# microsoft/singleshotpose

Hardware: NVIDIA H100
Metric: images/sec fwd+bwd+SGD (416x416, yolo-pose.cfg) (higher is better)
Workload: dtype f16x2-split operands, f32 accumulate (fwd); f16 operands, f32 accumulate (bwd)

## Files before the change

singleshotpose_b200/csrc/conv_tc.cu:

```cuda
#include "ssp_common.cuh"
#include "tmap.cuh"

namespace ssp {

struct ConvTcParams {
  CUtensorMap tmA[2];
  CUtensorMap tmB[2];
  long long m_rows;
  long long store_rows;
  int m_tiles, n_tiles;
  int kc_per_tap, cin, taps;
  int shifts[9];
  int Wp, HpWp;
  int cout, bn, n_terms;
  int fmt;
  int stages, stage_bytes, b_bytes;
  float* out;
  long long out_ld;
  const float* bias;
  double* stat_sum;
  double* stat_sq;
  int epi;
  FusedAct fa;
  int splits;
  long long slab_elems;
};

static constexpr int kABytes = 128 * 128;
static constexpr int kMaxStages = 8;
static constexpr int kAccCols = 1024;
static constexpr int kThreads = 256;
static constexpr int kSplitMinKblocks = 8;

template <bool FUSED, int BN, int BF, int NT, bool SPLIT = false>
__global__ void __launch_bounds__(kThreads, 1) conv_tc_kernel(const __grid_constant__ ConvTcParams p) {
  extern __shared__ __align__(1024) uint8_t smem_raw[];
  uint8_t* smem = (uint8_t*)(((uintptr_t)smem_raw + 1023) & ~(uintptr_t)1023);
  uint8_t* stage_base = smem;
  double* acc_sum = (double*)(smem + (size_t)p.stages * p.stage_bytes);
  double* acc_sq = acc_sum + kAccCols;
  float* stg = (float*)(acc_sq + kAccCols);
  uint64_t* full_bar = (uint64_t*)((uint8_t*)stg + kStageRowsBytes);
  uint64_t* empty_bar = full_bar + kMaxStages;

  const int warp = threadIdx.x >> 5;
  const int lane = threadIdx.x & 31;
  const int total_tiles = p.m_tiles * p.n_tiles;
  const int kblocks = p.taps * p.kc_per_tap;

  if (warp == 0 && lane == 0) {
    tma_prefetch_desc(&p.tmA[0]);
    tma_prefetch_desc(&p.tmB[0]);
    if (p.n_terms == 3) { tma_prefetch_desc(&p.tmA[1]); tma_prefetch_desc(&p.tmB[1]); }
  }
  if (warp == 1 && lane == 0) {
    for (int s = 0; s < p.stages; s++) { mbar_init(&full_bar[s], 1); mbar_init(&empty_bar[s], 4); }
    fence_barrier_init();
  }
  if (p.epi == EPI_STATS)
    for (int i = threadIdx.x; i < 2 * kAccCols; i += kThreads) acc_sum[i] = 0.0;
  __syncthreads();

  if (warp == 0) {
    if (lane == 0) {
      int stage = 0; uint32_t phase = 0;
      const uint32_t tx = (uint32_t)(p.n_terms == 3 ? 2 : 1) * (uint32_t)(kABytes + p.b_bytes);
      if constexpr (SPLIT) {
        for (int t = blockIdx.x; t < total_tiles * p.splits; t += gridDim.x) {
          const int tile = t / p.splits, sp = t % p.splits;
          const int m0 = (tile / p.n_tiles) * 128, n0 = (tile % p.n_tiles) * p.bn;
          const int kb1 = (int)((long long)(sp + 1) * kblocks / p.splits);
          for (int kb = (int)((long long)sp * kblocks / p.splits); kb < kb1; kb++) {
            const int tap = kb / p.kc_per_tap, kc = kb - tap * p.kc_per_tap;
            const int arow = m0 + p.shifts[tap];
            mbar_wait(&empty_bar[stage], phase ^ 1);
            uint8_t* sa = stage_base + (size_t)stage * p.stage_bytes;
            mbar_expect_tx(&full_bar[stage], tx);
            const int kcol_b = tap * p.cin + kc * 64;
            tma_load_2d(sa, &p.tmA[0], &full_bar[stage], kc * 64, arow);
            if (p.n_terms == 3) {
              tma_load_2d(sa + kABytes, &p.tmA[1], &full_bar[stage], kc * 64, arow);
              tma_load_2d(sa + 2 * kABytes, &p.tmB[0], &full_bar[stage], kcol_b, n0);
              tma_load_2d(sa + 2 * kABytes + p.b_bytes, &p.tmB[1], &full_bar[stage], kcol_b, n0);
            } else {
              tma_load_2d(sa + kABytes, &p.tmB[0], &full_bar[stage], kcol_b, n0);
            }
            if (++stage == p.stages) { stage = 0; phase ^= 1; }
          }
        }
      } else {
      for (int t = blockIdx.x; t < total_tiles; t += gridDim.x) {
        const int mt = t / p.n_tiles, nt = t % p.n_tiles;
        const int m0 = mt * 128, n0 = nt * p.bn;
        for (int tap = 0; tap < p.taps; tap++) {
          const int arow = m0 + p.shifts[tap];
          for (int kc = 0; kc < p.kc_per_tap; kc++) {
            mbar_wait(&empty_bar[stage], phase ^ 1);
            uint8_t* sa = stage_base + (size_t)stage * p.stage_bytes;
            mbar_expect_tx(&full_bar[stage], tx);
            const int kcol_b = tap * p.cin + kc * 64;
            tma_load_2d(sa, &p.tmA[0], &full_bar[stage], kc * 64, arow);
            if (p.n_terms == 3) {
              tma_load_2d(sa + kABytes, &p.tmA[1], &full_bar[stage], kc * 64, arow);
              tma_load_2d(sa + 2 * kABytes, &p.tmB[0], &full_bar[stage], kcol_b, n0);
              tma_load_2d(sa + 2 * kABytes + p.b_bytes, &p.tmB[1], &full_bar[stage], kcol_b, n0);
            } else {
              tma_load_2d(sa + kABytes, &p.tmB[0], &full_bar[stage], kcol_b, n0);
            }
            if (++stage == p.stages) { stage = 0; phase ^= 1; }
          }
        }
      }
      }
    }
  } else if (warp >= 4) {
    const int et = threadIdx.x - 128;
    int stage = 0; uint32_t phase = 0;
    float acc[2][BN / 2];
    const int items = SPLIT ? total_tiles * p.splits : total_tiles;
    for (int t = blockIdx.x; t < items; t += gridDim.x) {
      int tile = t, sp = 0, kb0 = 0, kb1 = kblocks;
      if constexpr (SPLIT) {
        tile = t / p.splits; sp = t % p.splits;
        kb0 = (int)((long long)sp * kblocks / p.splits); kb1 = (int)((long long)(sp + 1) * kblocks / p.splits);
      }
      const int mt = tile / p.n_tiles, nt = tile % p.n_tiles;
      int prev = -1;
      for (int kb = kb0; kb < kb1; kb++) {
        mbar_wait(&full_bar[stage], phase);
        const uint32_t sa = smem_u32(stage_base + (size_t)stage * p.stage_bytes);
        const uint32_t a_hi = sa, a_lo = sa + kABytes;
        const uint32_t b_hi = (NT == 3) ? sa + 2 * kABytes : sa + kABytes;
        const uint32_t b_lo = b_hi + p.b_bytes;
        wgmma_fence();
#pragma unroll
        for (int k = 0; k < 4; k++) {
          const uint64_t dbh = gmma_desc_k_sw128(b_hi + k * 32);
#pragma unroll
          for (int h = 0; h < 2; h++) {
            const uint64_t dah = gmma_desc_k_sw128(a_hi + h * 8192 + k * 32);
            const int sd = (kb > kb0 || k > 0) ? 1 : 0;
            if constexpr (NT == 3) {
              wgmma_f32<BN, 0, 0, BF>(acc[h], gmma_desc_k_sw128(a_lo + h * 8192 + k * 32), dbh, sd);
              wgmma_f32<BN, 0, 0, BF>(acc[h], dah, gmma_desc_k_sw128(b_lo + k * 32), 1);
              wgmma_f32<BN, 0, 0, BF>(acc[h], dah, dbh, 1);
            } else {
              wgmma_f32<BN, 0, 0, BF>(acc[h], dah, dbh, sd);
            }
          }
        }
        wgmma_commit();
        wgmma_wait<1>();
        if (prev >= 0 && lane == 0) mbar_arrive(&empty_bar[prev]);
        prev = stage;
        if (++stage == p.stages) { stage = 0; phase ^= 1; }
      }
      wgmma_wait<0>();
      if (prev >= 0 && lane == 0) mbar_arrive(&empty_bar[prev]);

      const long long m = (long long)mt * 128 + et;
      const int n0 = nt * p.bn;
      bool valid = false;
      if (m < p.m_rows) {
        const int rem = (int)(m % p.HpWp);
        valid = (rem / p.Wp >= 1) && (rem % p.Wp >= 1);
      }
      float* orow = (p.out && p.epi != EPI_F16) ? p.out + m * p.out_ld : nullptr;
      const bool can_store = m < p.store_rows;
#pragma unroll
      for (int ch = 0; ch < BN / 32; ch++) {
        float v[32];
        acc_rows_32<BN>(acc, ch, stg, et, v);
        const int c0 = n0 + ch * 32;
        if constexpr (SPLIT) {
          if (can_store) {
            float* o = p.out + sp * p.slab_elems + m * p.out_ld;
            if (c0 + 32 <= p.cout) {
#pragma unroll
              for (int j = 0; j < 32; j += 4) *reinterpret_cast<float4*>(o + c0 + j) = make_float4(v[j], v[j + 1], v[j + 2], v[j + 3]);
            } else {
#pragma unroll
              for (int j = 0; j < 32; j++) if (c0 + j < p.cout) o[c0 + j] = v[j];
            }
          }
          continue;
        }
        if constexpr (FUSED) {
          if (valid && c0 + 32 <= p.cout) {
            uint32_t ph[16], pl[16];
#pragma unroll
            for (int j = 0; j < 32; j += 2) {
              uint16_t h0, l0, h1, l1;
              float z0 = fmaf(v[j], __ldg(p.fa.scale + c0 + j), __ldg(p.fa.shift + c0 + j));
              float z1 = fmaf(v[j + 1], __ldg(p.fa.scale + c0 + j + 1), __ldg(p.fa.shift + c0 + j + 1));
              z0 = z0 > 0.f ? z0 : z0 * p.fa.slope; z1 = z1 > 0.f ? z1 : z1 * p.fa.slope;
              split_f16(z0, h0, l0); split_f16(z1, h1, l1);
              ph[j >> 1] = h0 | ((uint32_t)h1 << 16); pl[j >> 1] = l0 | ((uint32_t)l1 << 16);
            }
            uint4* dh = reinterpret_cast<uint4*>(p.fa.d_hi + m * p.fa.d_ld + p.fa.d_c0 + c0);
            uint4* dl = reinterpret_cast<uint4*>(p.fa.d_lo + m * p.fa.d_ld + p.fa.d_c0 + c0);
#pragma unroll
            for (int j = 0; j < 4; j++) {
              dh[j] = make_uint4(ph[4 * j], ph[4 * j + 1], ph[4 * j + 2], ph[4 * j + 3]);
              dl[j] = make_uint4(pl[4 * j], pl[4 * j + 1], pl[4 * j + 2], pl[4 * j + 3]);
            }
          }
          continue;
        }
        if (p.epi == EPI_BIAS) {
#pragma unroll
          for (int j = 0; j < 32; j++) if (c0 + j < p.cout) v[j] += __ldg(p.bias + c0 + j);
        }
        if (p.epi == EPI_F16) {
          if (can_store) {
            uint16_t* o16 = reinterpret_cast<uint16_t*>(p.out) + m * p.out_ld + c0;
            if (c0 + 32 <= p.cout) {
              uint32_t pk[16];
#pragma unroll
              for (int j = 0; j < 16; j++) pk[j] = cvt_f32_to_16(v[2 * j], FMT_F16) | ((uint32_t)cvt_f32_to_16(v[2 * j + 1], FMT_F16) << 16);
#pragma unroll
              for (int j = 0; j < 4; j++) reinterpret_cast<uint4*>(o16)[j] = make_uint4(pk[4 * j], pk[4 * j + 1], pk[4 * j + 2], pk[4 * j + 3]);
            } else {
#pragma unroll
              for (int j = 0; j < 32; j++) if (c0 + j < p.cout) o16[j] = cvt_f32_to_16(v[j], FMT_F16);
            }
          }
        } else if (can_store && p.epi != 3) {
          if (c0 + 32 <= p.cout) {
#pragma unroll
            for (int j = 0; j < 32; j += 4)
              *reinterpret_cast<float4*>(orow + c0 + j) = make_float4(v[j], v[j + 1], v[j + 2], v[j + 3]);
          } else {
#pragma unroll
            for (int j = 0; j < 32; j++) if (c0 + j < p.cout) orow[c0 + j] = v[j];
          }
        }
        if (p.epi == EPI_STATS) {
          float s1[32], s2[32];
#pragma unroll
          for (int j = 0; j < 32; j++) { const float x = valid ? v[j] : 0.f; s1[j] = x; s2[j] = x * x; }
          const float cs = warp_transpose_sum32(s1, lane);
          const float cq = warp_transpose_sum32(s2, lane);
          if (c0 + lane < p.cout) {
            atomicAdd(&acc_sum[c0 + lane], (double)cs);
            atomicAdd(&acc_sq[c0 + lane], (double)cq);
          }
        }
      }
    }
    if (p.epi == EPI_STATS) {
      epi_bar();
      for (int c = et; c < p.cout; c += 128) {
        const double a = acc_sum[c], b = acc_sq[c];
        if (a != 0.0 || b != 0.0) { atomicAdd(p.stat_sum + c, a); atomicAdd(p.stat_sq + c, b); }
      }
    }
  }
}

template <bool FUSED, int BF, int NT, bool SPLIT = false>
static int launch_conv_tc(const ConvTcParams& p, int grid, int smem_bytes, cudaStream_t stream) {
  static int configured = 0;
  if (!configured) {
    cudaError_t e = cudaSuccess;
    for (auto k : {conv_tc_kernel<FUSED, 32, BF, NT, SPLIT>, conv_tc_kernel<FUSED, 64, BF, NT, SPLIT>, conv_tc_kernel<FUSED, 128, BF, NT, SPLIT>})
      if (e == cudaSuccess) e = cudaFuncSetAttribute(k, cudaFuncAttributeMaxDynamicSharedMemorySize, 227 * 1024);
    if (e != cudaSuccess) return fail_cuda(e, __FILE__, __LINE__);
    configured = 1;
  }
  if (p.bn == 32) conv_tc_kernel<FUSED, 32, BF, NT, SPLIT><<<grid, kThreads, smem_bytes, stream>>>(p);
  else if (p.bn == 64) conv_tc_kernel<FUSED, 64, BF, NT, SPLIT><<<grid, kThreads, smem_bytes, stream>>>(p);
  else conv_tc_kernel<FUSED, 128, BF, NT, SPLIT><<<grid, kThreads, smem_bytes, stream>>>(p);
  SSP_CHECK_LAUNCH();
  return SSP_OK;
}

static int g_num_sms = 0;

static void tile_geometry(int N, int H, int W, int taps, int cin, int cout, long long* tiles, int* kblocks) {
  const int bn = cout > 64 ? 128 : ((cout + 31) / 32) * 32;
  *tiles = ((Geom{N, H, W}.m_rows() + 127) / 128) * (long long)((cout + bn - 1) / bn);
  *kblocks = taps * ((cin + 63) / 64);
}

int conv_splitk_count(int N, int H, int W, int taps, int cin, int cout, int num_sms) {
  if (N <= 0 || H <= 0 || W <= 0 || (taps != 1 && taps != 9) || cin <= 0 || cout <= 0 || num_sms <= 0)
    return fail_msg(SSP_ERR_ARG, "ssp_conv_splitk_count: bad argument");
  long long tiles; int kblocks;
  tile_geometry(N, H, W, taps, cin, cout, &tiles, &kblocks);
  long long s = num_sms / tiles;
  if (s > kblocks / kSplitMinKblocks) s = kblocks / kSplitMinKblocks;
  return s < 2 ? 1 : (int)s;
}

int conv_gemm_tc(const void* a_hi, const void* a_lo, long long a_rows, int a_ld, int cin,
                 const void* b_hi, const void* b_lo, int b_rows, int b_ld, int a_fmt, int b_fmt,
                 int N, int H, int W, int taps, int cout, float* out, int out_ld, long long out_rows,
                 int epi, const float* bias, double* stat_sum, double* stat_sq, cudaStream_t stream, const FusedAct* fa,
                 const SplitK* sk) {
  if (sk) {
    long long tiles; int kblocks;
    tile_geometry(N, H, W, taps, cin, cout, &tiles, &kblocks);
    if (fa || epi != EPI_F32) return fail_msg(SSP_ERR_ARG, "conv_gemm_tc: split-K stores plain fp32 partial sums");
    if (sk->splits < 1 || (cin > 0 && (taps == 1 || taps == 9) && sk->splits > kblocks))
      return fail_msg(SSP_ERR_ARG, "ssp_conv_gemm_splitk: splits must be in [1, k-blocks] (taps * ceil(cin / 64))");
    if (!out || ((uintptr_t)out % 16) || (out_ld % 4) || out_ld < cout || (sk->slab_elems % 4))
      return fail_msg(SSP_ERR_ARG, "ssp_conv_gemm_splitk: workspace must be non-null and 16-B aligned, partial_ld % 4 == 0 and >= cout, slab_elems % 4 == 0");
    if (sk->slab_elems < flat_alloc_rows(N, H, W) * (long long)out_ld)
      return fail_msg(SSP_ERR_ARG, "ssp_conv_gemm_splitk: a slab must hold ssp_flat_alloc_rows(N, H, W) * partial_ld elements");
    out_rows = flat_alloc_rows(N, H, W);
  }
  if (fa) {
    if (!fa->scale || !fa->shift || !fa->d_hi || !fa->d_lo || (cout % 32) || (fa->d_ld % 8) || (fa->d_c0 % 8))
      return fail_msg(SSP_ERR_ARG, "conv_gemm_tc: fused BN+activation epilogue needs cout % 32 == 0 and 16-B aligned destination rows");
    epi = EPI_BNACT;
  }
  if (!a_hi || !b_hi || (!out && !fa) || (taps != 1 && taps != 9) || cin <= 0 || cout <= 0) return fail_msg(SSP_ERR_ARG, "conv_gemm_tc: bad argument");
  if ((a_ld % 8) || (b_ld % 8)) return fail_msg(SSP_ERR_ARG, "conv_gemm_tc: leading dimensions must be multiples of 8 elements (16 B)");
  if (epi == EPI_STATS && (cout > kAccCols || !stat_sum || !stat_sq)) return fail_msg(SSP_ERR_ARG, "conv_gemm_tc: statistics need cout <= 1024 and buffers");
  if (epi == EPI_BIAS && !bias) return fail_msg(SSP_ERR_ARG, "conv_gemm_tc: bias missing");
  if (!fa && epi != EPI_F16 && ((out_ld % 4) || ((uintptr_t)out % 16))) return fail_msg(SSP_ERR_ARG, "conv_gemm_tc: output must be 16-B aligned with ld % 4 == 0");
  if (epi == EPI_F16 && ((out_ld % 8) || ((uintptr_t)out % 16))) return fail_msg(SSP_ERR_ARG, "conv_gemm_tc: fp16 output must be 16-B aligned with ld % 8 == 0");
  if (a_fmt != b_fmt) return fail_msg(SSP_ERR_ARG, "conv_gemm_tc: both operands must have the same 16-bit format");
  if (!g_num_sms) {
    g_num_sms = ssp_sm_count();
  }
  ConvTcParams p;
  Geom g{N, H, W};
  p.n_terms = (a_lo && b_lo) ? 3 : 1;
  int bn = ((cout + 31) / 32) * 32;
  if (bn > 64) bn = 128;
  p.bn = bn;
  p.b_bytes = bn * 128;
  p.m_rows = g.m_rows();
  p.store_rows = out_rows;
  p.m_tiles = (int)((p.m_rows + 127) / 128);
  p.n_tiles = (cout + bn - 1) / bn;
  p.kc_per_tap = (cin + 63) / 64;
  p.cin = cin;
  p.taps = taps;
  for (int t = 0; t < 9; t++) p.shifts[t] = (taps == 9) ? ((t / 3) - 1) * g.Wp() + ((t % 3) - 1) : 0;
  p.Wp = g.Wp(); p.HpWp = g.HpWp();
  p.cout = cout;
  p.fmt = a_fmt;
  p.stage_bytes = (p.n_terms == 3 ? 2 : 1) * (kABytes + p.b_bytes);
  const int fixed = 2 * kAccCols * 8 + kStageRowsBytes + 2 * kMaxStages * 8 + 1024;
  int stages = (227 * 1024 - fixed) / p.stage_bytes;
  if (stages > kMaxStages) stages = kMaxStages;
  if (stages < 2) return fail_msg(SSP_ERR_ARG, "conv_gemm_tc: tile does not fit shared memory");
  p.stages = stages;
  p.out = out; p.out_ld = out_ld; p.bias = bias; p.stat_sum = stat_sum; p.stat_sq = stat_sq; p.epi = epi;
  if (fa) p.fa = *fa; else p.fa = FusedAct{nullptr, nullptr, 1.f, nullptr, nullptr, 0, 0};
  p.splits = sk ? sk->splits : 1;
  p.slab_elems = sk ? sk->slab_elems : 0;
  int rc = 0;
  rc |= tmap_2d_16bit(&p.tmA[0], a_hi, (uint64_t)cin, (uint64_t)a_rows, (uint64_t)a_ld, 64, 128, a_fmt == FMT_BF16);
  rc |= tmap_2d_16bit(&p.tmB[0], b_hi, (uint64_t)taps * cin, (uint64_t)b_rows, (uint64_t)b_ld, 64, bn, b_fmt == FMT_BF16);
  if (p.n_terms == 3) {
    rc |= tmap_2d_16bit(&p.tmA[1], a_lo, (uint64_t)cin, (uint64_t)a_rows, (uint64_t)a_ld, 64, 128, a_fmt == FMT_BF16);
    rc |= tmap_2d_16bit(&p.tmB[1], b_lo, (uint64_t)taps * cin, (uint64_t)b_rows, (uint64_t)b_ld, 64, bn, b_fmt == FMT_BF16);
  }
  if (rc) return fail_msg(SSP_ERR_DRIVER, "conv_gemm_tc: cuTensorMapEncodeTiled failed (no driver, or misaligned operand)");
  const int smem_bytes = stages * p.stage_bytes + fixed;
  const int total = p.m_tiles * p.n_tiles;
  const int grid = total < g_num_sms ? total : g_num_sms;
  if (p.n_terms == 3 && p.fmt == FMT_BF16) return fail_msg(SSP_ERR_ARG, "conv_gemm_tc: split (hi/lo) operands must be fp16");
  if (sk) {
    const long long items = (long long)total * sk->splits;
    const int sgrid = items < g_num_sms ? (int)items : g_num_sms;
    return p.n_terms == 3 ? launch_conv_tc<false, 0, 3, true>(p, sgrid, smem_bytes, stream) : launch_conv_tc<false, 0, 1, true>(p, sgrid, smem_bytes, stream);
  }
  if (fa) return p.n_terms == 3 ? launch_conv_tc<true, 0, 3>(p, grid, smem_bytes, stream) : launch_conv_tc<true, 0, 1>(p, grid, smem_bytes, stream);
  if (p.n_terms == 3) return launch_conv_tc<false, 0, 3>(p, grid, smem_bytes, stream);
  return p.fmt == FMT_BF16 ? launch_conv_tc<false, 1, 1>(p, grid, smem_bytes, stream) : launch_conv_tc<false, 0, 1>(p, grid, smem_bytes, stream);
}

}
```

singleshotpose_b200/csrc/ssp_common.cuh:

```cuda
#pragma once
#include <cuda_runtime.h>
#include <cuda_fp16.h>
#include <cuda_bf16.h>
#include <stdint.h>
#include <stdlib.h>

#include "../../include/ssp_b200.h"

#define SSP_CHECK_LAUNCH()                                   \
  do {                                                       \
    cudaError_t e__ = cudaGetLastError();                    \
    if (e__ != cudaSuccess) return ssp::fail_cuda(e__, __FILE__, __LINE__); \
  } while (0)

namespace ssp {

int fail_cuda(cudaError_t e, const char* file, int line);
int fail_msg(int code, const char* msg);

inline int ssp_sm_count() {
  static int n = 0;
  if (!n) {
    int dev = 0; cudaGetDevice(&dev);
    cudaDeviceGetAttribute(&n, cudaDevAttrMultiProcessorCount, dev);
    const char* e = getenv("SSP_SM_LIMIT");
    if (e) { const int l = atoi(e) & ~1; if (l >= 2 && l < n) n = l; }
  }
  return n;
}
enum Fmt16 { FMT_F16 = 0, FMT_BF16 = 1 };
enum { EPI_F32 = 0, EPI_STATS = 1, EPI_BIAS = 2, EPI_BNACT = 4, EPI_F16 = 8 };
struct FusedAct {
  const float* scale; const float* shift; float slope;
  uint16_t* d_hi; uint16_t* d_lo; long long d_ld; int d_c0;
};
struct SplitK { int splits; long long slab_elems; };
struct Geom {
  int N, H, W;
  __host__ __device__ int Wp() const { return W + 1; }
  __host__ __device__ int HpWp() const { return (H + 1) * (W + 1); }
  __host__ __device__ long long m_rows() const { return (long long)N * (H + 1) * (W + 1); }
  __host__ __device__ long long row(int n, int h, int w) const {
    return (long long)n * HpWp() + (long long)(h + 1) * Wp() + (w + 1);
  }
};

__host__ __device__ inline long long flat_alloc_rows(int N, int H, int W) {
  long long m = (long long)N * (H + 1) * (W + 1) + (W + 1) + 2;
  return ((m + 127) / 128) * 128 + 128;
}

__device__ __forceinline__ float cvt16_to_f32(uint16_t v, int fmt) {
  return fmt == FMT_F16 ? __half2float(__ushort_as_half(v)) : __bfloat162float(__ushort_as_bfloat16(v));
}
__device__ __forceinline__ uint16_t cvt_f32_to_16(float f, int fmt) {
  return fmt == FMT_F16 ? __half_as_ushort(__float2half_rn(fminf(fmaxf(f, -65504.f), 65504.f)))
                        : __bfloat16_as_ushort(__float2bfloat16_rn(f));
}
__device__ __forceinline__ void split_f16(float f, uint16_t& hi, uint16_t& lo) {
  __half h = __float2half_rn(f);
  hi = __half_as_ushort(h);
  lo = __half_as_ushort(__float2half_rn(f - __half2float(h)));
}

__device__ __forceinline__ uint32_t smem_u32(const void* p) {
  return static_cast<uint32_t>(__cvta_generic_to_shared(p));
}
__device__ __forceinline__ void mbar_init(uint64_t* bar, uint32_t count) {
  asm volatile("mbarrier.init.shared::cta.b64 [%0], %1;" ::"r"(smem_u32(bar)), "r"(count) : "memory");
}
__device__ __forceinline__ void fence_barrier_init() {
  asm volatile("fence.mbarrier_init.release.cluster;" ::: "memory");
}
__device__ __forceinline__ void fence_proxy_async() {
  asm volatile("fence.proxy.async.shared::cta;" ::: "memory");
}
__device__ __forceinline__ void mbar_expect_tx(uint64_t* bar, uint32_t bytes) {
  asm volatile("mbarrier.arrive.expect_tx.shared::cta.b64 _, [%0], %1;" ::"r"(smem_u32(bar)), "r"(bytes) : "memory");
}
__device__ __forceinline__ void mbar_arrive(uint64_t* bar) {
  asm volatile("mbarrier.arrive.shared::cta.b64 _, [%0];" ::"r"(smem_u32(bar)) : "memory");
}
__device__ __forceinline__ bool mbar_try_wait(uint64_t* bar, uint32_t parity) {
  uint32_t ok;
  asm volatile(
      "{\n\t.reg .pred p;\n\t"
      "mbarrier.try_wait.parity.shared::cta.b64 p, [%1], %2;\n\t"
      "selp.u32 %0, 1, 0, p;\n\t}"
      : "=r"(ok)
      : "r"(smem_u32(bar)), "r"(parity)
      : "memory");
  return ok != 0;
}
__device__ __forceinline__ void mbar_wait(uint64_t* bar, uint32_t parity) {
  uint32_t spins = 0;
  while (!mbar_try_wait(bar, parity)) {
    if (++spins > (1u << 26)) { __trap(); }
  }
}
__device__ __forceinline__ void tma_load_2d(void* smem_dst, const void* tmap, uint64_t* bar, int c0, int c1) {
  asm volatile(
      "cp.async.bulk.tensor.2d.shared::cluster.global.tile.mbarrier::complete_tx::bytes [%0], [%1, {%3, %4}], [%2];"
      ::"r"(smem_u32(smem_dst)), "l"(tmap), "r"(smem_u32(bar)), "r"(c0), "r"(c1)
      : "memory");
}
__device__ __forceinline__ void tma_prefetch_desc(const void* tmap) {
  asm volatile("prefetch.tensormap [%0];" ::"l"(tmap) : "memory");
}
__device__ __forceinline__ void epi_bar() { asm volatile("bar.sync 1, 128;" ::: "memory"); }

__device__ __forceinline__ uint64_t gmma_desc_sw128(uint32_t smem_addr, uint32_t lbo_bytes, uint32_t sbo_bytes) {
  uint64_t d = 0;
  d |= (uint64_t)((smem_addr >> 4) & 0x3FFF);
  d |= (uint64_t)((lbo_bytes >> 4) & 0x3FFF) << 16;
  d |= (uint64_t)((sbo_bytes >> 4) & 0x3FFF) << 32;
  d |= (uint64_t)1 << 62;
  return d;
}
__device__ __forceinline__ uint64_t gmma_desc_k_sw128(uint32_t smem_addr) { return gmma_desc_sw128(smem_addr, 16, 1024); }
__device__ __forceinline__ void wgmma_fence() { asm volatile("wgmma.fence.sync.aligned;" ::: "memory"); }
__device__ __forceinline__ void wgmma_commit() { asm volatile("wgmma.commit_group.sync.aligned;" ::: "memory"); }
template <int N>
__device__ __forceinline__ void wgmma_wait() { asm volatile("wgmma.wait_group.sync.aligned %0;" ::"n"(N) : "memory"); }

template <int TA, int TB>
__device__ __forceinline__ void wgmma_m64n32k16_f16(float (&d)[16], uint64_t da, uint64_t db, int sd) {
  asm volatile(
      "{\n\t.reg .pred p;\n\tsetp.ne.b32 p, %18, 0;\n\t"
      "wgmma.mma_async.sync.aligned.m64n32k16.f32.f16.f16 {%0, %1, %2, %3, %4, %5, %6, %7, %8, %9, %10, %11, %12, %13, %14, %15}, %16, %17, p, 1, 1, %19, %20;\n\t}"
      : "+f"(d[0]), "+f"(d[1]), "+f"(d[2]), "+f"(d[3]), "+f"(d[4]), "+f"(d[5]), "+f"(d[6]), "+f"(d[7]), "+f"(d[8]), "+f"(d[9]), "+f"(d[10]), "+f"(d[11]), "+f"(d[12]), "+f"(d[13]), "+f"(d[14]), "+f"(d[15])
      : "l"(da), "l"(db), "r"(sd), "n"(TA), "n"(TB));
}
template <int TA, int TB>
__device__ __forceinline__ void wgmma_m64n32k16_bf16(float (&d)[16], uint64_t da, uint64_t db, int sd) {
  asm volatile(
      "{\n\t.reg .pred p;\n\tsetp.ne.b32 p, %18, 0;\n\t"
      "wgmma.mma_async.sync.aligned.m64n32k16.f32.bf16.bf16 {%0, %1, %2, %3, %4, %5, %6, %7, %8, %9, %10, %11, %12, %13, %14, %15}, %16, %17, p, 1, 1, %19, %20;\n\t}"
      : "+f"(d[0]), "+f"(d[1]), "+f"(d[2]), "+f"(d[3]), "+f"(d[4]), "+f"(d[5]), "+f"(d[6]), "+f"(d[7]), "+f"(d[8]), "+f"(d[9]), "+f"(d[10]), "+f"(d[11]), "+f"(d[12]), "+f"(d[13]), "+f"(d[14]), "+f"(d[15])
      : "l"(da), "l"(db), "r"(sd), "n"(TA), "n"(TB));
}
template <int TA, int TB>
__device__ __forceinline__ void wgmma_m64n64k16_f16(float (&d)[32], uint64_t da, uint64_t db, int sd) {
  asm volatile(
      "{\n\t.reg .pred p;\n\tsetp.ne.b32 p, %34, 0;\n\t"
      "wgmma.mma_async.sync.aligned.m64n64k16.f32.f16.f16 {%0, %1, %2, %3, %4, %5, %6, %7, %8, %9, %10, %11, %12, %13, %14, %15, %16, %17, %18, %19, %20, %21, %22, %23, %24, %25, %26, %27, %28, %29, %30, %31}, %32, %33, p, 1, 1, %35, %36;\n\t}"
      : "+f"(d[0]), "+f"(d[1]), "+f"(d[2]), "+f"(d[3]), "+f"(d[4]), "+f"(d[5]), "+f"(d[6]), "+f"(d[7]), "+f"(d[8]), "+f"(d[9]), "+f"(d[10]), "+f"(d[11]), "+f"(d[12]), "+f"(d[13]), "+f"(d[14]), "+f"(d[15]), "+f"(d[16]), "+f"(d[17]), "+f"(d[18]), "+f"(d[19]), "+f"(d[20]), "+f"(d[21]), "+f"(d[22]), "+f"(d[23]), "+f"(d[24]), "+f"(d[25]), "+f"(d[26]), "+f"(d[27]), "+f"(d[28]), "+f"(d[29]), "+f"(d[30]), "+f"(d[31])
      : "l"(da), "l"(db), "r"(sd), "n"(TA), "n"(TB));
}
template <int TA, int TB>
__device__ __forceinline__ void wgmma_m64n64k16_bf16(float (&d)[32], uint64_t da, uint64_t db, int sd) {
  asm volatile(
      "{\n\t.reg .pred p;\n\tsetp.ne.b32 p, %34, 0;\n\t"
      "wgmma.mma_async.sync.aligned.m64n64k16.f32.bf16.bf16 {%0, %1, %2, %3, %4, %5, %6, %7, %8, %9, %10, %11, %12, %13, %14, %15, %16, %17, %18, %19, %20, %21, %22, %23, %24, %25, %26, %27, %28, %29, %30, %31}, %32, %33, p, 1, 1, %35, %36;\n\t}"
      : "+f"(d[0]), "+f"(d[1]), "+f"(d[2]), "+f"(d[3]), "+f"(d[4]), "+f"(d[5]), "+f"(d[6]), "+f"(d[7]), "+f"(d[8]), "+f"(d[9]), "+f"(d[10]), "+f"(d[11]), "+f"(d[12]), "+f"(d[13]), "+f"(d[14]), "+f"(d[15]), "+f"(d[16]), "+f"(d[17]), "+f"(d[18]), "+f"(d[19]), "+f"(d[20]), "+f"(d[21]), "+f"(d[22]), "+f"(d[23]), "+f"(d[24]), "+f"(d[25]), "+f"(d[26]), "+f"(d[27]), "+f"(d[28]), "+f"(d[29]), "+f"(d[30]), "+f"(d[31])
      : "l"(da), "l"(db), "r"(sd), "n"(TA), "n"(TB));
}
template <int TA, int TB>
__device__ __forceinline__ void wgmma_m64n128k16_f16(float (&d)[64], uint64_t da, uint64_t db, int sd) {
  asm volatile(
      "{\n\t.reg .pred p;\n\tsetp.ne.b32 p, %66, 0;\n\t"
      "wgmma.mma_async.sync.aligned.m64n128k16.f32.f16.f16 {%0, %1, %2, %3, %4, %5, %6, %7, %8, %9, %10, %11, %12, %13, %14, %15, %16, %17, %18, %19, %20, %21, %22, %23, %24, %25, %26, %27, %28, %29, %30, %31, %32, %33, %34, %35, %36, %37, %38, %39, %40, %41, %42, %43, %44, %45, %46, %47, %48, %49, %50, %51, %52, %53, %54, %55, %56, %57, %58, %59, %60, %61, %62, %63}, %64, %65, p, 1, 1, %67, %68;\n\t}"
      : "+f"(d[0]), "+f"(d[1]), "+f"(d[2]), "+f"(d[3]), "+f"(d[4]), "+f"(d[5]), "+f"(d[6]), "+f"(d[7]), "+f"(d[8]), "+f"(d[9]), "+f"(d[10]), "+f"(d[11]), "+f"(d[12]), "+f"(d[13]), "+f"(d[14]), "+f"(d[15]), "+f"(d[16]), "+f"(d[17]), "+f"(d[18]), "+f"(d[19]), "+f"(d[20]), "+f"(d[21]), "+f"(d[22]), "+f"(d[23]), "+f"(d[24]), "+f"(d[25]), "+f"(d[26]), "+f"(d[27]), "+f"(d[28]), "+f"(d[29]), "+f"(d[30]), "+f"(d[31]), "+f"(d[32]), "+f"(d[33]), "+f"(d[34]), "+f"(d[35]), "+f"(d[36]), "+f"(d[37]), "+f"(d[38]), "+f"(d[39]), "+f"(d[40]), "+f"(d[41]), "+f"(d[42]), "+f"(d[43]), "+f"(d[44]), "+f"(d[45]), "+f"(d[46]), "+f"(d[47]), "+f"(d[48]), "+f"(d[49]), "+f"(d[50]), "+f"(d[51]), "+f"(d[52]), "+f"(d[53]), "+f"(d[54]), "+f"(d[55]), "+f"(d[56]), "+f"(d[57]), "+f"(d[58]), "+f"(d[59]), "+f"(d[60]), "+f"(d[61]), "+f"(d[62]), "+f"(d[63])
      : "l"(da), "l"(db), "r"(sd), "n"(TA), "n"(TB));
}
template <int TA, int TB>
__device__ __forceinline__ void wgmma_m64n128k16_bf16(float (&d)[64], uint64_t da, uint64_t db, int sd) {
  asm volatile(
      "{\n\t.reg .pred p;\n\tsetp.ne.b32 p, %66, 0;\n\t"
      "wgmma.mma_async.sync.aligned.m64n128k16.f32.bf16.bf16 {%0, %1, %2, %3, %4, %5, %6, %7, %8, %9, %10, %11, %12, %13, %14, %15, %16, %17, %18, %19, %20, %21, %22, %23, %24, %25, %26, %27, %28, %29, %30, %31, %32, %33, %34, %35, %36, %37, %38, %39, %40, %41, %42, %43, %44, %45, %46, %47, %48, %49, %50, %51, %52, %53, %54, %55, %56, %57, %58, %59, %60, %61, %62, %63}, %64, %65, p, 1, 1, %67, %68;\n\t}"
      : "+f"(d[0]), "+f"(d[1]), "+f"(d[2]), "+f"(d[3]), "+f"(d[4]), "+f"(d[5]), "+f"(d[6]), "+f"(d[7]), "+f"(d[8]), "+f"(d[9]), "+f"(d[10]), "+f"(d[11]), "+f"(d[12]), "+f"(d[13]), "+f"(d[14]), "+f"(d[15]), "+f"(d[16]), "+f"(d[17]), "+f"(d[18]), "+f"(d[19]), "+f"(d[20]), "+f"(d[21]), "+f"(d[22]), "+f"(d[23]), "+f"(d[24]), "+f"(d[25]), "+f"(d[26]), "+f"(d[27]), "+f"(d[28]), "+f"(d[29]), "+f"(d[30]), "+f"(d[31]), "+f"(d[32]), "+f"(d[33]), "+f"(d[34]), "+f"(d[35]), "+f"(d[36]), "+f"(d[37]), "+f"(d[38]), "+f"(d[39]), "+f"(d[40]), "+f"(d[41]), "+f"(d[42]), "+f"(d[43]), "+f"(d[44]), "+f"(d[45]), "+f"(d[46]), "+f"(d[47]), "+f"(d[48]), "+f"(d[49]), "+f"(d[50]), "+f"(d[51]), "+f"(d[52]), "+f"(d[53]), "+f"(d[54]), "+f"(d[55]), "+f"(d[56]), "+f"(d[57]), "+f"(d[58]), "+f"(d[59]), "+f"(d[60]), "+f"(d[61]), "+f"(d[62]), "+f"(d[63])
      : "l"(da), "l"(db), "r"(sd), "n"(TA), "n"(TB));
}

template <int N, int TA, int TB, int BF16>
__device__ __forceinline__ void wgmma_f32(float (&d)[N / 2], uint64_t da, uint64_t db, int sd) {
  if constexpr (N == 32) { if constexpr (BF16) wgmma_m64n32k16_bf16<TA, TB>(d, da, db, sd); else wgmma_m64n32k16_f16<TA, TB>(d, da, db, sd); }
  else if constexpr (N == 64) { if constexpr (BF16) wgmma_m64n64k16_bf16<TA, TB>(d, da, db, sd); else wgmma_m64n64k16_f16<TA, TB>(d, da, db, sd); }
  else { static_assert(N == 128, "N in {32, 64, 128}"); if constexpr (BF16) wgmma_m64n128k16_bf16<TA, TB>(d, da, db, sd); else wgmma_m64n128k16_f16<TA, TB>(d, da, db, sd); }
}

static constexpr int kStageRowsBytes = 128 * 33 * 4;
template <int N, int HALVES = 2>
__device__ __forceinline__ void acc_stage_32(const float (&acc)[2][N / 2], int ch, float* stg, int t) {
  const int w = t >> 5, l = t & 31;
  epi_bar();
#pragma unroll
  for (int c = 0; c < N / 32; c++) {
    if (c == ch) {
#pragma unroll
      for (int h = 0; h < HALVES; h++)
#pragma unroll
        for (int j = 0; j < 16; j++) {
          const int i = 16 * c + j;
          const int row = h * 64 + w * 16 + (l >> 2) + 8 * ((i >> 1) & 1);
          const int col = ((i >> 2) & 3) * 8 + (l & 3) * 2 + (i & 1);
          stg[row * 33 + col] = acc[h][i];
        }
    }
  }
  epi_bar();
}
template <int N, int HALVES = 2>
__device__ __forceinline__ void acc_rows_32(const float (&acc)[2][N / 2], int ch, float* stg, int t, float (&v)[32]) {
  acc_stage_32<N, HALVES>(acc, ch, stg, t);
  if (t < HALVES * 64) {
#pragma unroll
    for (int j = 0; j < 32; j++) v[j] = stg[t * 33 + j];
  }
}

__device__ __forceinline__ uint32_t cluster_ctarank() { uint32_t r; asm volatile("mov.u32 %0, %%cluster_ctarank;" : "=r"(r)); return r; }
__device__ __forceinline__ void cluster_sync_all() {
  asm volatile("barrier.cluster.arrive.release.aligned;\n\tbarrier.cluster.wait.acquire.aligned;" ::: "memory");
}
__device__ __forceinline__ void fence_cluster() { asm volatile("fence.acq_rel.cluster;" ::: "memory"); }
__device__ __forceinline__ void mbar_arrive_remote(uint64_t* bar, uint32_t rank) {
  asm volatile("{\n\t.reg .b32 ra;\n\tmapa.shared::cluster.u32 ra, %0, %1;\n\tmbarrier.arrive.release.cluster.shared::cluster.b64 _, [ra];\n\t}"
               ::"r"(smem_u32(bar)), "r"(rank) : "memory");
}
__device__ __forceinline__ float ld_remote_f32(const float* p, uint32_t rank) {
  float v;
  asm volatile("{\n\t.reg .b32 ra;\n\tmapa.shared::cluster.u32 ra, %1, %2;\n\tld.shared::cluster.f32 %0, [ra];\n\t}"
               : "=f"(v) : "r"(smem_u32(p)), "r"(rank) : "memory");
  return v;
}
__device__ __forceinline__ void mbar_wait_cluster(uint64_t* bar, uint32_t parity) {
  uint32_t spins = 0;
  for (;;) {
    uint32_t ok;
    asm volatile(
        "{\n\t.reg .pred p;\n\t"
        "mbarrier.try_wait.parity.acquire.cluster.shared::cta.b64 p, [%1], %2;\n\t"
        "selp.u32 %0, 1, 0, p;\n\t}"
        : "=r"(ok) : "r"(smem_u32(bar)), "r"(parity) : "memory");
    if (ok) return;
    if (++spins > (1u << 26)) { __trap(); }
  }
}

__device__ __forceinline__ void sgd_update(float& p, float g, float& v, float lr, float mu, float wd, float gscale) {
  const float vn = fmaf(mu, v, fmaf(wd, p, g * gscale));
  v = vn;
  p = fmaf(-lr, vn, p);
}

template <int OFF>
__device__ __forceinline__ void warp_transpose_level(float (&v)[32], int lane) {
  const bool up = (lane & OFF) != 0;
#pragma unroll
  for (int i = 0; i < OFF; i++) {
    const float send = up ? v[i] : v[i + OFF];
    const float keep = up ? v[i + OFF] : v[i];
    v[i] = keep + __shfl_xor_sync(0xffffffffu, send, OFF);
  }
  if constexpr (OFF > 1) warp_transpose_level<OFF / 2>(v, lane);
}
__device__ __forceinline__ float warp_transpose_sum32(float (&v)[32], int lane) {
  warp_transpose_level<16>(v, lane);
  return v[0];
}

}
```

Measured before the change: 1642.

## Add ping-pong consumer warpgroups with register reallocation to conv_tc kernel

Expands the kernel to 384 threads: one producer warpgroup that gives up registers via setmaxnreg, and two consumer warpgroups that take alternate tiles in ping-pong order, handing off through named barriers. The goal is to overlap one warpgroup's epilogue with the other's WGMMA main loop. Per-CTA shared-memory stats accumulation is removed in favour of direct global double atomics, and the epilogue staging shrinks to 16-column chunks so each consumer gets its own staging buffer. Risks include extra named-barrier synchronisation, more global atomic traffic, register pressure at 240 regs per consumer, and ping-pong only being enabled when there are more tiles than CTAs.

```diff
diff --git a/singleshotpose_b200/csrc/conv_tc.cu b/singleshotpose_b200/csrc/conv_tc.cu
--- a/singleshotpose_b200/csrc/conv_tc.cu
+++ b/singleshotpose_b200/csrc/conv_tc.cu
@@ -24,29 +24,55 @@
   FusedAct fa;
   int splits;
   long long slab_elems;
+  int pingpong;
 };
 
 static constexpr int kABytes = 128 * 128;
 static constexpr int kMaxStages = 8;
-static constexpr int kAccCols = 1024;
-static constexpr int kThreads = 256;
+static constexpr int kThreads = 384;
+static constexpr int kProducerRegs = 24, kConsumerRegs = 240;
+static constexpr int kStage16Bytes = 128 * 17 * 4;
+static constexpr int kBarEpi = 1, kBarTurn = 3;
 static constexpr int kSplitMinKblocks = 8;
+
+template <int N>
+__device__ __forceinline__ void acc_rows_16(const float (&acc)[2][N / 2], int ch, int q, float* stg, int t, int bar, float* v) {
+  const int w = t >> 5, l = t & 31;
+  named_bar_sync(bar, 128);
+#pragma unroll
+  for (int c = 0; c < N / 32; c++) {
+    if (c == ch) {
+#pragma unroll
+      for (int h = 0; h < 2; h++)
+#pragma unroll
+        for (int j = 8 * q; j < 8 * q + 8; j++) {
+          const int i = 16 * c + j;
+          const int row = h * 64 + w * 16 + (l >> 2) + 8 * ((i >> 1) & 1);
+          const int col = ((i >> 2) & 1) * 8 + (l & 3) * 2 + (i & 1);
+          stg[row * 17 + col] = acc[h][i];
+        }
+    }
+  }
+  named_bar_sync(bar, 128);
+#pragma unroll
+  for (int j = 0; j < 16; j++) v[j] = stg[t * 17 + j];
+}
 
 template <bool FUSED, int BN, int BF, int NT, bool SPLIT = false>
 __global__ void __launch_bounds__(kThreads, 1) conv_tc_kernel(const __grid_constant__ ConvTcParams p) {
   extern __shared__ __align__(1024) uint8_t smem_raw[];
   uint8_t* smem = (uint8_t*)(((uintptr_t)smem_raw + 1023) & ~(uintptr_t)1023);
   uint8_t* stage_base = smem;
-  double* acc_sum = (double*)(smem + (size_t)p.stages * p.stage_bytes);
-  double* acc_sq = acc_sum + kAccCols;
-  float* stg = (float*)(acc_sq + kAccCols);
-  uint64_t* full_bar = (uint64_t*)((uint8_t*)stg + kStageRowsBytes);
+  float* stg_base = (float*)(smem + (size_t)p.stages * p.stage_bytes);
+  uint64_t* full_bar = (uint64_t*)((uint8_t*)stg_base + 2 * kStage16Bytes);
   uint64_t* empty_bar = full_bar + kMaxStages;
 
   const int warp = threadIdx.x >> 5;
   const int lane = threadIdx.x & 31;
+  const int wg = threadIdx.x >> 7;
   const int total_tiles = p.m_tiles * p.n_tiles;
   const int kblocks = p.taps * p.kc_per_tap;
+  const int items = SPLIT ? total_tiles * p.splits : total_tiles;
 
   if (warp == 0 && lane == 0) {
     tma_prefetch_desc(&p.tmA[0]);
@@ -57,12 +83,11 @@
     for (int s = 0; s < p.stages; s++) { mbar_init(&full_bar[s], 1); mbar_init(&empty_bar[s], 4); }
     fence_barrier_init();
   }
-  if (p.epi == EPI_STATS)
-    for (int i = threadIdx.x; i < 2 * kAccCols; i += kThreads) acc_sum[i] = 0.0;
   __syncthreads();
 
-  if (warp == 0) {
-    if (lane == 0) {
+  if (wg == 0) {
+    setmaxnreg_dec<kProducerRegs>();
+    if (warp == 0 && lane == 0) {
       int stage = 0; uint32_t phase = 0;
       const uint32_t tx = (uint32_t)(p.n_terms == 3 ? 2 : 1) * (uint32_t)(kABytes + p.b_bytes);
       if constexpr (SPLIT) {
@@ -73,7 +98,7 @@
           for (int kb = (int)((long long)sp * kblocks / p.splits); kb < kb1; kb++) {
             const int tap = kb / p.kc_per_tap, kc = kb - tap * p.kc_per_tap;
             const int arow = m0 + p.shifts[tap];
-            mbar_wait(&empty_bar[stage], phase ^ 1);
+            mbar_wait_regs(&empty_bar[stage], phase ^ 1);
             uint8_t* sa = stage_base + (size_t)stage * p.stage_bytes;
             mbar_expect_tx(&full_bar[stage], tx);
             const int kcol_b = tap * p.cin + kc * 64;
@@ -95,7 +120,7 @@
         for (int tap = 0; tap < p.taps; tap++) {
           const int arow = m0 + p.shifts[tap];
           for (int kc = 0; kc < p.kc_per_tap; kc++) {
-            mbar_wait(&empty_bar[stage], phase ^ 1);
+            mbar_wait_regs(&empty_bar[stage], phase ^ 1);
             uint8_t* sa = stage_base + (size_t)stage * p.stage_bytes;
             mbar_expect_tx(&full_bar[stage], tx);
             const int kcol_b = tap * p.cin + kc * 64;
@@ -113,21 +138,28 @@
       }
       }
     }
-  } else if (warp >= 4) {
-    const int et = threadIdx.x - 128;
-    int stage = 0; uint32_t phase = 0;
+  } else {
+    setmaxnreg_inc<kConsumerRegs>();
+    const int cw = wg - 1;
+    const int et = threadIdx.x - 128 * wg;
+    float* stg = stg_base + cw * (kStage16Bytes / 4);
     float acc[2][BN / 2];
-    const int items = SPLIT ? total_tiles * p.splits : total_tiles;
-    for (int t = blockIdx.x; t < items; t += gridDim.x) {
+    int pos = 0;
+    for (int i = 0; blockIdx.x + (long long)i * gridDim.x < items; i++) {
+      const int t = blockIdx.x + i * gridDim.x;
       int tile = t, sp = 0, kb0 = 0, kb1 = kblocks;
       if constexpr (SPLIT) {
         tile = t / p.splits; sp = t % p.splits;
         kb0 = (int)((long long)sp * kblocks / p.splits); kb1 = (int)((long long)(sp + 1) * kblocks / p.splits);
       }
+      if (p.pingpong ? (i & 1) != cw : cw != 0) { pos += kb1 - kb0; continue; }
+      if (p.pingpong && i > 0) named_bar_sync(kBarTurn + cw, 256);
+      int stage = pos % p.stages; uint32_t phase = (pos / p.stages) & 1;
+      pos += kb1 - kb0;
       const int mt = tile / p.n_tiles, nt = tile % p.n_tiles;
       int prev = -1;
       for (int kb = kb0; kb < kb1; kb++) {
-        mbar_wait(&full_bar[stage], phase);
+        mbar_wait_regs(&full_bar[stage], phase);
         const uint32_t sa = smem_u32(stage_base + (size_t)stage * p.stage_bytes);
         const uint32_t a_hi = sa, a_lo = sa + kABytes;
         const uint32_t b_hi = (NT == 3) ? sa + 2 * kABytes : sa + kABytes;
@@ -155,6 +187,7 @@
         prev = stage;
         if (++stage == p.stages) { stage = 0; phase ^= 1; }
       }
+      if (p.pingpong && blockIdx.x + (long long)(i + 1) * gridDim.x < items) named_bar_arrive(kBarTurn + (cw ^ 1), 256);
       wgmma_wait<0>();
       if (prev >= 0 && lane == 0) mbar_arrive(&empty_bar[prev]);
 
@@ -169,9 +202,38 @@
       const bool can_store = m < p.store_rows;
 #pragma unroll
       for (int ch = 0; ch < BN / 32; ch++) {
+        const int c0 = n0 + ch * 32;
+        if constexpr (FUSED) {
+#pragma unroll
+          for (int q = 0; q < 2; q++) {
+            float v[16];
+            acc_rows_16<BN>(acc, ch, q, stg, et, kBarEpi + cw, v);
+            if (valid && c0 + 32 <= p.cout) {
+              const int c = c0 + 16 * q;
+              uint32_t ph[8], pl[8];
+#pragma unroll
+              for (int j = 0; j < 16; j += 2) {
+                uint16_t h0, l0, h1, l1;
+                float z0 = fmaf(v[j], __ldg(p.fa.scale + c + j), __ldg(p.fa.shift + c + j));
+                float z1 = fmaf(v[j + 1], __ldg(p.fa.scale + c + j + 1), __ldg(p.fa.shift + c + j + 1));
+                z0 = z0 > 0.f ? z0 : z0 * p.fa.slope; z1 = z1 > 0.f ? z1 : z1 * p.fa.slope;
+                split_f16(z0, h0, l0); split_f16(z1, h1, l1);
+                ph[j >> 1] = h0 | ((uint32_t)h1 << 16); pl[j >> 1] = l0 | ((uint32_t)l1 << 16);
+              }
+              uint4* dh = reinterpret_cast<uint4*>(p.fa.d_hi + m * p.fa.d_ld + p.fa.d_c0 + c);
+              uint4* dl = reinterpret_cast<uint4*>(p.fa.d_lo + m * p.fa.d_ld + p.fa.d_c0 + c);
+#pragma unroll
+              for (int j = 0; j < 2; j++) {
+                dh[j] = make_uint4(ph[4 * j], ph[4 * j + 1], ph[4 * j + 2], ph[4 * j + 3]);
+                dl[j] = make_uint4(pl[4 * j], pl[4 * j + 1], pl[4 * j + 2], pl[4 * j + 3]);
+              }
+            }
+          }
+          continue;
+        }
         float v[32];
-        acc_rows_32<BN>(acc, ch, stg, et, v);
-        const int c0 = n0 + ch * 32;
+        acc_rows_16<BN>(acc, ch, 0, stg, et, kBarEpi + cw, v);
+        acc_rows_16<BN>(acc, ch, 1, stg, et, kBarEpi + cw, v + 16);
         if constexpr (SPLIT) {
           if (can_store) {
             float* o = p.out + sp * p.slab_elems + m * p.out_ld;
@@ -181,28 +243,6 @@
             } else {
 #pragma unroll
               for (int j = 0; j < 32; j++) if (c0 + j < p.cout) o[c0 + j] = v[j];
-            }
-          }
-          continue;
-        }
-        if constexpr (FUSED) {
-          if (valid && c0 + 32 <= p.cout) {
-            uint32_t ph[16], pl[16];
-#pragma unroll
-            for (int j = 0; j < 32; j += 2) {
-              uint16_t h0, l0, h1, l1;
-              float z0 = fmaf(v[j], __ldg(p.fa.scale + c0 + j), __ldg(p.fa.shift + c0 + j));
-              float z1 = fmaf(v[j + 1], __ldg(p.fa.scale + c0 + j + 1), __ldg(p.fa.shift + c0 + j + 1));
-              z0 = z0 > 0.f ? z0 : z0 * p.fa.slope; z1 = z1 > 0.f ? z1 : z1 * p.fa.slope;
-              split_f16(z0, h0, l0); split_f16(z1, h1, l1);
-              ph[j >> 1] = h0 | ((uint32_t)h1 << 16); pl[j >> 1] = l0 | ((uint32_t)l1 << 16);
-            }
-            uint4* dh = reinterpret_cast<uint4*>(p.fa.d_hi + m * p.fa.d_ld + p.fa.d_c0 + c0);
-            uint4* dl = reinterpret_cast<uint4*>(p.fa.d_lo + m * p.fa.d_ld + p.fa.d_c0 + c0);
-#pragma unroll
-            for (int j = 0; j < 4; j++) {
-              dh[j] = make_uint4(ph[4 * j], ph[4 * j + 1], ph[4 * j + 2], ph[4 * j + 3]);
-              dl[j] = make_uint4(pl[4 * j], pl[4 * j + 1], pl[4 * j + 2], pl[4 * j + 3]);
             }
           }
           continue;
@@ -242,17 +282,10 @@
           const float cs = warp_transpose_sum32(s1, lane);
           const float cq = warp_transpose_sum32(s2, lane);
           if (c0 + lane < p.cout) {
-            atomicAdd(&acc_sum[c0 + lane], (double)cs);
-            atomicAdd(&acc_sq[c0 + lane], (double)cq);
-          }
-        }
-      }
-    }
-    if (p.epi == EPI_STATS) {
-      epi_bar();
-      for (int c = et; c < p.cout; c += 128) {
-        const double a = acc_sum[c], b = acc_sq[c];
-        if (a != 0.0 || b != 0.0) { atomicAdd(p.stat_sum + c, a); atomicAdd(p.stat_sq + c, b); }
+            atomicAdd(p.stat_sum + c0 + lane, (double)cs);
+            atomicAdd(p.stat_sq + c0 + lane, (double)cq);
+          }
+        }
       }
     }
   }
@@ -276,6 +309,11 @@
 }
 
 static int g_num_sms = 0;
+
+static constexpr int kPingPongMaxKblocks = 143;
+static int pingpong_schedule(long long items, int grid, int kblocks) {
+  return (items > grid && kblocks <= kPingPongMaxKblocks) ? 1 : 0;
+}
 
 static void tile_geometry(int N, int H, int W, int taps, int cin, int cout, long long* tiles, int* kblocks) {
   const int bn = cout > 64 ? 128 : ((cout + 31) / 32) * 32;
@@ -317,7 +355,7 @@
   }
   if (!a_hi || !b_hi || (!out && !fa) || (taps != 1 && taps != 9) || cin <= 0 || cout <= 0) return fail_msg(SSP_ERR_ARG, "conv_gemm_tc: bad argument");
   if ((a_ld % 8) || (b_ld % 8)) return fail_msg(SSP_ERR_ARG, "conv_gemm_tc: leading dimensions must be multiples of 8 elements (16 B)");
-  if (epi == EPI_STATS && (cout > kAccCols || !stat_sum || !stat_sq)) return fail_msg(SSP_ERR_ARG, "conv_gemm_tc: statistics need cout <= 1024 and buffers");
+  if (epi == EPI_STATS && (!stat_sum || !stat_sq)) return fail_msg(SSP_ERR_ARG, "conv_gemm_tc: statistics need buffers");
   if (epi == EPI_BIAS && !bias) return fail_msg(SSP_ERR_ARG, "conv_gemm_tc: bias missing");
   if (!fa && epi != EPI_F16 && ((out_ld % 4) || ((uintptr_t)out % 16))) return fail_msg(SSP_ERR_ARG, "conv_gemm_tc: output must be 16-B aligned with ld % 4 == 0");
   if (epi == EPI_F16 && ((out_ld % 8) || ((uintptr_t)out % 16))) return fail_msg(SSP_ERR_ARG, "conv_gemm_tc: fp16 output must be 16-B aligned with ld % 8 == 0");
@@ -344,7 +382,7 @@
   p.cout = cout;
   p.fmt = a_fmt;
   p.stage_bytes = (p.n_terms == 3 ? 2 : 1) * (kABytes + p.b_bytes);
-  const int fixed = 2 * kAccCols * 8 + kStageRowsBytes + 2 * kMaxStages * 8 + 1024;
+  const int fixed = 2 * kStage16Bytes + 2 * kMaxStages * 8 + 1024;
   int stages = (227 * 1024 - fixed) / p.stage_bytes;
   if (stages > kMaxStages) stages = kMaxStages;
   if (stages < 2) return fail_msg(SSP_ERR_ARG, "conv_gemm_tc: tile does not fit shared memory");
@@ -364,10 +402,12 @@
   const int smem_bytes = stages * p.stage_bytes + fixed;
   const int total = p.m_tiles * p.n_tiles;
   const int grid = total < g_num_sms ? total : g_num_sms;
+  p.pingpong = pingpong_schedule(total, grid, p.taps * p.kc_per_tap);
   if (p.n_terms == 3 && p.fmt == FMT_BF16) return fail_msg(SSP_ERR_ARG, "conv_gemm_tc: split (hi/lo) operands must be fp16");
   if (sk) {
     const long long items = (long long)total * sk->splits;
     const int sgrid = items < g_num_sms ? (int)items : g_num_sms;
+    p.pingpong = pingpong_schedule(items, sgrid, p.taps * p.kc_per_tap / sk->splits);
     return p.n_terms == 3 ? launch_conv_tc<false, 0, 3, true>(p, sgrid, smem_bytes, stream) : launch_conv_tc<false, 0, 1, true>(p, sgrid, smem_bytes, stream);
   }
   if (fa) return p.n_terms == 3 ? launch_conv_tc<true, 0, 3>(p, grid, smem_bytes, stream) : launch_conv_tc<true, 0, 1>(p, grid, smem_bytes, stream);
diff --git a/singleshotpose_b200/csrc/ssp_common.cuh b/singleshotpose_b200/csrc/ssp_common.cuh
--- a/singleshotpose_b200/csrc/ssp_common.cuh
+++ b/singleshotpose_b200/csrc/ssp_common.cuh
@@ -98,6 +98,13 @@
     if (++spins > (1u << 26)) { __trap(); }
   }
 }
+static __device__ __noinline__ void mbar_wait_timeout() { __trap(); }
+__device__ __forceinline__ void mbar_wait_regs(uint64_t* bar, uint32_t parity) {
+  uint32_t spins = 0;
+  while (!mbar_try_wait(bar, parity)) {
+    if (++spins > (1u << 26)) mbar_wait_timeout();
+  }
+}
 __device__ __forceinline__ void tma_load_2d(void* smem_dst, const void* tmap, uint64_t* bar, int c0, int c1) {
   asm volatile(
       "cp.async.bulk.tensor.2d.shared::cluster.global.tile.mbarrier::complete_tx::bytes [%0], [%1, {%3, %4}], [%2];"
@@ -108,6 +115,10 @@
   asm volatile("prefetch.tensormap [%0];" ::"l"(tmap) : "memory");
 }
 __device__ __forceinline__ void epi_bar() { asm volatile("bar.sync 1, 128;" ::: "memory"); }
+__device__ __forceinline__ void named_bar_sync(int id, int n) { asm volatile("bar.sync %0, %1;" ::"r"(id), "r"(n) : "memory"); }
+__device__ __forceinline__ void named_bar_arrive(int id, int n) { asm volatile("bar.arrive %0, %1;" ::"r"(id), "r"(n) : "memory"); }
+template <int R> __device__ __forceinline__ void setmaxnreg_inc() { asm volatile("setmaxnreg.inc.sync.aligned.u32 %0;" ::"n"(R)); }
+template <int R> __device__ __forceinline__ void setmaxnreg_dec() { asm volatile("setmaxnreg.dec.sync.aligned.u32 %0;" ::"n"(R)); }
 
 __device__ __forceinline__ uint64_t gmma_desc_sw128(uint32_t smem_addr, uint32_t lbo_bytes, uint32_t sbo_bytes) {
   uint64_t d = 0;
```

New measurement: 1674 (median of 6 runs). About the same (+2.0%).
